# YuxiaWu/RAG4DyG

Hardware: AMD Instinct MI355X
Metric: query-seqs/sec encode+top-k over full pool (higher is better)
Workload: dtype f32 (f16x2 operands: two fp16 terms, three products, f32 accumulate)

## Files before the change

### rag4dyg_amd/build.py

```python
import os
import subprocess
import sys
from concurrent.futures import ThreadPoolExecutor

PKG = os.path.dirname(os.path.abspath(__file__))
CSRC = os.path.join(PKG, "csrc")
OBJ = os.path.join(PKG, "_build")
LIB = os.path.join(PKG, "librag4dyg_hip.so")
HIPCC = os.environ.get("HIPCC", "/opt/rocm/bin/hipcc")
FLAGS = ["-O3", "--offload-arch=gfx950", "-fPIC", "-std=c++17", "-Wall", "-Wno-unused-function"]


def sources():
    return sorted(os.path.join(CSRC, f) for f in os.listdir(CSRC) if f.endswith(".hip"))


def _deps_mtime():
    hdrs = [os.path.join(CSRC, f) for f in os.listdir(CSRC) if f.endswith(".h")]
    hdrs.append(os.path.join(os.path.dirname(PKG), "include", "r4d.h"))
    return max(os.path.getmtime(h) for h in hdrs)


def _compile(src, force, hdr_m):
    obj = os.path.join(OBJ, os.path.basename(src)[:-4] + ".o")
    if not force and os.path.exists(obj) and os.path.getmtime(obj) >= max(os.path.getmtime(src), hdr_m):
        return obj, False
    cmd = [HIPCC, *FLAGS, "-c", src, "-o", obj]
    r = subprocess.run(cmd, capture_output=True, text=True)
    if r.returncode != 0:
        raise RuntimeError(f"hipcc failed for {src}:\n{r.stdout}\n{r.stderr}")
    if r.stderr.strip():
        sys.stderr.write(r.stderr)
    return obj, True


HANDOFF_KERNELS = {"topk.hip": {"topk_chunk_kernelIfE": (4, 2), "topk_chunk_kernelIdE": (4, 2)},
                   "gemm_skinny.hip": {"gemm_skinny16_kernelILi2ELi0E": (2, 1), "gemm_skinny16_kernelILi3ELi0E": (2, 1)}}


def check_handoff_lowering(src):
    import re
    import tempfile
    names = HANDOFF_KERNELS[os.path.basename(src)]
    with tempfile.TemporaryDirectory() as td:
        asm = os.path.join(td, "k.s")
        r = subprocess.run([HIPCC, "-O3", "--offload-arch=gfx950", "-std=c++17", "--offload-device-only", "-S", src, "-o", asm],
                           capture_output=True, text=True)
        if r.returncode != 0:
            raise RuntimeError(f"hipcc -S failed for {src}:\n{r.stderr}")
        text = open(asm).read()
    for name, (want_st, want_ld) in names.items():
        m = re.search(r"^(_ZN3r4d\d+" + re.escape(name) + r"[^\n:]*):[^\n]*\n(.*?)s_endpgm", text, re.S | re.M)
        if not m:
            raise RuntimeError(f"hand-off check: kernel {name} not found in the assembly of {src}")
        body = m.group(2)
        stores = re.findall(r"global_store_dword(?:x2)? [^\n]*", body)
        loads_sc1 = [ln for ln in re.findall(r"global_load_dword(?:x2)? [^\n]*", body) if " sc1" in ln]
        stores_sc1 = [ln for ln in stores if " sc1" in ln]
        ticket = re.findall(r"global_atomic_add[^\n]*", body)
        if not ticket or len(stores_sc1) < want_st or len(loads_sc1) < want_ld:
            raise RuntimeError(f"hand-off check FAILED for {name}: {len(stores_sc1)} sc1 stores (want {want_st}), {len(loads_sc1)} sc1 loads (want {want_ld}), "
                               f"{len(ticket)} ticket atomics -- the relaxed agent-scope publish / consume of {os.path.basename(src)} "
                               "is no longer lowered to write-through / L1-bypassing instructions; use release / acquire there")


PACKED_F32_FILES = ("gemm_h2.hip", "attention_h2.hip")
PACKED_F32_FORMS = {
    "v_pk_mul_f32 V, V, S op_sel_hi:[1,0]", "v_pk_mul_f32 V, S, V op_sel_hi:[0,1]", "v_pk_mul_f32 V, V, S", "v_pk_mul_f32 V, S, V",
    "v_pk_fma_f32 V, V, S, V op_sel_hi:[1,0,1]", "v_pk_fma_f32 V, S, V, V op_sel_hi:[0,1,1]", "v_pk_fma_f32 V, V, S, V", "v_pk_fma_f32 V, S, V, V",
    "v_pk_fma_f32 V, V, S, V op_sel_hi:[1,0,1] neg_lo:[0,0,1] neg_hi:[0,0,1]",
    "v_pk_fma_f32 V, V, S, V op_sel_hi:[1,0,0] neg_lo:[1,0,0] neg_hi:[1,0,0]",
    "v_pk_fma_f32 V, S, V, V op_sel_hi:[0,1,1] neg_lo:[1,0,0] neg_hi:[1,0,0]",
    "v_pk_add_f32 V, V, S op_sel_hi:[1,0]", "v_pk_add_f32 V, S, V op_sel_hi:[0,1]",
}


def check_packed_f32_forms(src):
    import re
    import tempfile
    with tempfile.TemporaryDirectory() as td:
        asm = os.path.join(td, "k.s")
        r = subprocess.run([HIPCC, "-O3", "--offload-arch=gfx950", "-std=c++17", "--offload-device-only", "-S", src, "-o", asm],
                           capture_output=True, text=True)
        if r.returncode != 0:
            raise RuntimeError(f"hipcc -S failed for {src}:\n{r.stderr}")
        text = open(asm).read()
    seen = {}
    for ln in re.findall(r"^\s*(v_pk_(?:fma|mul|add)_f32 [^\n;]*)", text, re.M):
        if not re.search(r"\bs\[?\d", ln):
            continue
        form = re.sub(r"a\[[0-9:]+\]", "V", re.sub(r"v\[[0-9:]+\]", "V", re.sub(r"\bs\[[0-9:]+\]|\bs\d+\b", "S", ln))).strip()
        seen[form] = seen.get(form, 0) + 1
    new = {f: n for f, n in seen.items() if f not in PACKED_F32_FORMS}
    if new:
        raise RuntimeError(f"packed-fp32 census FAILED for {os.path.basename(src)}: operand forms with an SGPR source that "
                           f"tools/pk_fma_probe.hip has not verified on gfx950: {new} -- add the form to the probe, run it on the GPU, "
                           "then list it in rag4dyg_amd/build.py:PACKED_F32_FORMS (or pin that arithmetic scalar)")
    return seen


def build_library(force=False, verbose=True):
    os.makedirs(OBJ, exist_ok=True)
    hdr_m = _deps_mtime()
    with ThreadPoolExecutor(max_workers=4) as ex:
        res = list(ex.map(lambda s: _compile(s, force, hdr_m), sources()))
    objs = [o for o, _ in res]
    for src, (_o, compiled) in zip(sources(), res):
        if compiled and os.path.basename(src) in HANDOFF_KERNELS:
            check_handoff_lowering(src)
        if compiled and os.path.basename(src) in PACKED_F32_FILES:
            check_packed_f32_forms(src)
    stale = os.path.exists(LIB) and any(os.path.getmtime(o) > os.path.getmtime(LIB) for o in objs)
    if force or stale or any(c for _, c in res) or not os.path.exists(LIB):
        cmd = [HIPCC, "--offload-arch=gfx950", "-shared", "-fPIC", "-o", LIB, *objs]
        r = subprocess.run(cmd, capture_output=True, text=True)
        if r.returncode != 0:
            raise RuntimeError(f"link failed:\n{r.stdout}\n{r.stderr}")
        if verbose:
            print(f"built {LIB}")
    elif verbose:
        print(f"up to date: {LIB}")
    return LIB


if __name__ == "__main__":
    build_library(force="--force" in sys.argv)
```

### rag4dyg_amd/csrc/gemm_h2p_body.h

```cpp
    constexpr int NW = WGM * WGN;
    constexpr int WM = BM / WGM, WN = BN / WGN, TM = WM / 32, TN = WN / 32;
    constexpr int STAGE = (BM + BN) * 8;
    constexpr int NBUF = 3;
    constexpr int NGA = BM / 8 / NW, NGB = BN / 8 / NW;
    constexpr int NDMA = NGA + NGB;
    static_assert(BM == 128 && (BN == 256 || BN == 128) && TM >= 1 && TN >= 1 && (NGA == 2 || NGA == 4) && (NGB == 2 || NGB == 4 || NGB == 8), "tile");
    __shared__ u32x4 lds[NBUF * STAGE];

    static_assert(!ROWMAP || (EPI == EPI_H2WORDS && !OUT_LINES), "row-block map: the h2-word c_attn only");
    int m0, n0;
    if constexpr (ROWMAP) {
        const int tiles_m = rm.hdr[0] >> 2, tiles_n = (g.N + BN - 1) / BN, nreal = tiles_m * tiles_n;
        if ((int)blockIdx.x >= nreal) return;
        grouped_tile<BM, BN>(tiles_m, tiles_n, (int)blockIdx.x, nreal, m0, n0);
    } else {
        grouped_tile<BM, BN>(g.M, g.N, m0, n0);
    }
    const int nkt = g.K / 32;

    const int tid = threadIdx.x, lane = tid & 63, wid = tid >> 6;
    const int wm = wid / WGN, wn = wid % WGN;
    const int li = lane & 31, lh = lane >> 5;

    unsigned va[NGA], vb[NGB];
    const int lrow = lane >> 3, lslot = lane & 7;
#pragma unroll
    for (int i = 0; i < NGA; ++i) {
        const int r = (wid * NGA + i) * 8 + lrow;
        int arow;
        if constexpr (ROWMAP) {
            const int gr = rm.list[(m0 + r) >> 5] * 32 + (r & 31);
            arow = gr >= rm.m_tab ? rm.m_tab - 1 : (gr >= rm.m_real && gr < ((rm.m_real + 31) & ~31) ? rm.m_real - 1 : gr);
        } else {
            arow = min(m0 + r, g.M - 1);
        }
        va[i] = (unsigned)arow * (unsigned)(g.K * 4) + 16u * (unsigned)(lslot ^ ((r >> 1) & 7)) + 3072u - 1024u * (i & 3);
    }
#pragma unroll
    for (int i = 0; i < NGB; ++i) {
        const int r = (wid * NGB + i) * 8 + lrow;
        vb[i] = (unsigned)min(n0 + r, g.N - 1) * (unsigned)(g.K * 4) + 16u * (unsigned)(lslot ^ ((r >> 1) & 7)) + 3072u - 1024u * (i & 3);
    }
    const unsigned lds0 = __builtin_amdgcn_readfirstlane((unsigned)(size_t)lds);
    const unsigned wid_s = __builtin_amdgcn_readfirstlane((unsigned)wid);
    const unsigned dst_a = lds0 + (wid_s * NGA) * 1024u, dst_b = lds0 + ((unsigned)(BM / 8) + wid_s * NGB) * 1024u;
    const char* abase = reinterpret_cast<const char*>(Al) - 3072;
    const char* bbase = reinterpret_cast<const char*>(Bp) - 3072;
#define H2P_ISSUE(KT, STG)                                                                         \
    {                                                                                              \
        const unsigned so_ = (unsigned)(STG) * (unsigned)(STAGE * 16);                             \
        if constexpr (NGA == 4) h2p_dma4(abase + (size_t)(KT) * 128, va[0], va[1], va[2], va[3], dst_a + so_); \
        else h2p_dma2(abase + (size_t)(KT) * 128, va[0], va[1], dst_a + so_);                      \
        if constexpr (NGB == 8) {                                                                  \
            h2p_dma4(bbase + (size_t)(KT) * 128, vb[0], vb[1], vb[2], vb[3], dst_b + so_);          \
            h2p_dma4(bbase + (size_t)(KT) * 128, vb[4], vb[5], vb[6], vb[7], dst_b + so_ + 4096u);   \
        } else if constexpr (NGB == 4) h2p_dma4(bbase + (size_t)(KT) * 128, vb[0], vb[1], vb[2], vb[3], dst_b + so_); \
        else h2p_dma2(bbase + (size_t)(KT) * 128, vb[0], vb[1], dst_b + so_);                       \
    }

    const int fsw = (li >> 1) & 7;
    int f_off[2][2];
#pragma unroll
    for (int s_ = 0; s_ < 2; ++s_)
#pragma unroll
        for (int p = 0; p < 2; ++p) f_off[s_][p] = li * 8 + ((4 * p + 2 * s_ + lh) ^ fsw);
    const int fa_base = wm * WM * 8, fb_base = BM * 8 + wn * WN * 8;

    f32x16 acc0[TM][TN], acc1[TM][TN];
#pragma unroll
    for (int i = 0; i < TM; ++i)
#pragma unroll
        for (int j = 0; j < TN; ++j)
#pragma unroll
            for (int r = 0; r < 16; ++r) { acc0[i][j][r] = 0.f; acc1[i][j][r] = 0.f; }

#define H2P_MFMA(ACC, A_, B_, I_, J_) \
    ACC[I_][J_] = __builtin_amdgcn_mfma_f32_32x32x16_f16(__builtin_bit_cast(f16x8, A_), __builtin_bit_cast(f16x8, B_), ACC[I_][J_], 0, 0, 0);
    u32x4 fa[2][TM][2], fb[2][TN][2];
#define H2P_FRAGS(SET, STG, S)                                                                     \
    {                                                                                              \
        const u32x4* st_ = lds + (STG) * STAGE;                                                   \
                                        \
        _Pragma("unroll") for (int i = 0; i < TM; ++i) fa[SET][i][1] = st_[fa_base + i * 256 + f_off[S][1]]; \
        _Pragma("unroll") for (int j = 0; j < TN; ++j) fb[SET][j][0] = st_[fb_base + j * 256 + f_off[S][0]]; \
        _Pragma("unroll") for (int i = 0; i < TM; ++i) fa[SET][i][0] = st_[fa_base + i * 256 + f_off[S][0]]; \
        _Pragma("unroll") for (int j = 0; j < TN; ++j) fb[SET][j][1] = st_[fb_base + j * 256 + f_off[S][1]]; \
    }
#define H2P_MFMAS(SET)                                                                             \
    {                                                                                              \
        _Pragma("unroll") for (int i = 0; i < TM; ++i) _Pragma("unroll") for (int j = 0; j < TN; ++j) H2P_MFMA(acc1, fa[SET][i][1], fb[SET][j][0], i, j) \
        _Pragma("unroll") for (int i = 0; i < TM; ++i) _Pragma("unroll") for (int j = 0; j < TN; ++j) H2P_MFMA(acc0, fa[SET][i][0], fb[SET][j][0], i, j) \
        _Pragma("unroll") for (int i = 0; i < TM; ++i) _Pragma("unroll") for (int j = 0; j < TN; ++j) H2P_MFMA(acc1, fa[SET][i][0], fb[SET][j][1], i, j) \
    }

    H2P_ISSUE(0, 0)
    if (nkt > 1) { H2P_ISSUE(1, 1) h2p_wait_vm<NDMA>(); } else { h2p_wait_vm<0>(); }
    __syncthreads();
    H2P_FRAGS(0, 0, 0)

    constexpr int NMF = 3 * TM * TN, NFR = 2 * (TM + TN);
    static_assert(NMF >= NFR, "interleave");
#define H2P_ITER(CUR, NXT, WR)                                                                     \
    {                                                                                              \
        __builtin_amdgcn_sched_barrier(0);                                                         \
        const bool more_ = kt + 2 < nkt;                                                           \
        if (more_) H2P_ISSUE(kt + 2, WR)                                                           \
        H2P_FRAGS(1, CUR, 1)                                                                       \
        H2P_MFMAS(0)                                                                               \
        _Pragma("unroll") for (int m_ = 0; m_ < NMF; ++m_) {                                       \
            __builtin_amdgcn_sched_group_barrier(0x008, 1, 0);                                     \
            if (m_ < NFR) __builtin_amdgcn_sched_group_barrier(0x100, 1, 0);                       \
        }                                                                                          \
        __builtin_amdgcn_sched_barrier(0);                                                         \
        if (more_) h2p_wait_vm<NDMA>(); else h2p_wait_vm<0>();                                     \
        asm volatile("s_waitcnt lgkmcnt(0)\n\ts_barrier" ::: "memory");                            \
        H2P_FRAGS(0, NXT, 0)                                                                       \
        H2P_MFMAS(1)                                                                               \
        _Pragma("unroll") for (int m_ = 0; m_ < NMF; ++m_) {                                       \
            __builtin_amdgcn_sched_group_barrier(0x008, 1, 0);                                     \
            if (m_ < NFR) __builtin_amdgcn_sched_group_barrier(0x100, 1, 0);                       \
        }                                                                                          \
        __builtin_amdgcn_sched_barrier(0);                                                         \
    }
    int kt = 0;
    for (; kt + 2 < nkt; kt += 3) {
        H2P_ITER(0, 1, 2)
        { ++kt; H2P_ITER(1, 2, 0) }
        { ++kt; H2P_ITER(2, 0, 1) }
        kt -= 2;
    }
    if (kt < nkt) {
        H2P_ITER(0, 1, 2)
        if (kt + 1 < nkt) { ++kt; H2P_ITER(1, 2, 0) }
    }
#undef H2P_ITER
#undef H2P_FRAGS
#undef H2P_MFMAS
#undef H2P_MFMA
#undef H2P_ISSUE

    constexpr float UNS = H2_A_UNSCALE;
    float* __restrict__ C = Cg;
    const bool interior = ROWMAP || ((m0 + BM <= g.M) & (n0 + BN <= g.N));
    if constexpr (OUT_LINES) {
        static_assert(EPI == EPI_GELU, "line output: the c_fc epilogue only");
        unsigned char* __restrict__ L = reinterpret_cast<unsigned char*>(Cg);
        const long long row_bytes = (long long)g.N * 4;
        const bool odd = li & 1;
#pragma unroll
        for (int j = 0; j < TN; ++j) {
            const int colb = n0 + wn * WN + j * 32;
            const bool col_ok = colb + li < g.N;
            const float bias = (biasg && col_ok) ? biasg[colb + li] : 0.f;
#pragma unroll
            for (int i = 0; i < TM; ++i) {
#pragma unroll
                for (int r2 = 0; r2 < 16; r2 += 2) {
                    f32x2 v2 = {__builtin_fmaf(acc1[i][j][r2], H2_LO_UNSCALE, acc0[i][j][r2]) * UNS + bias,
                                __builtin_fmaf(acc1[i][j][r2 + 1], H2_LO_UNSCALE, acc0[i][j][r2 + 1]) * UNS + bias};
                    v2 = gelu_new2(v2);
                    const float vx = v2.x, vy = v2.y;
                    const float send = odd ? vx : vy;
                    const float recv = __builtin_bit_cast(float, __builtin_amdgcn_mov_dpp(__builtin_bit_cast(int, send), 0xB1, 0xF, 0xF, true));
                    const float c0 = odd ? recv : vx, c1 = odd ? vy : recv;
                    unsigned h, l;
                    split2_pair<true>(c0, c1, h, l);
                    const int r = r2 + (odd ? 1 : 0);
                    const int row = m0 + wm * WM + i * 32 + (r & 3) + 8 * (r >> 2) + 4 * lh;
                    if (interior || (row < g.M && col_ok)) {
                        unsigned* dst = reinterpret_cast<unsigned*>(L + (long long)row * row_bytes + (long long)(colb >> 5) * 128 + (li >> 1) * 4);
                        dst[0] = h;
                        dst[16] = l;
                    }
                }
            }
        }
        return;
    } else {
        if (interior) {
            const int lane_c = (((ROWMAP ? 0 : wm * WM) + 4 * lh) * g.ldc + wn * WN + li) * 4;
            const int lane_r = ((wm * WM + 4 * lh) * g.ldr + wn * WN + li) * 4;
            const __amdgpu_buffer_rsrc_t c_rsrc = __builtin_amdgcn_make_buffer_rsrc(
                C + (long long)(ROWMAP ? 0 : m0) * g.ldc + n0, 0, (((ROWMAP ? g.M : BM) - 1) * g.ldc + BN) * 4, 0x00020000);
            const __amdgpu_buffer_rsrc_t r_rsrc = __builtin_amdgcn_make_buffer_rsrc(
                const_cast<float*>(EPI == EPI_RESIDUAL ? residg + (long long)m0 * g.ldr + n0 : Cg), 0,
                EPI == EPI_RESIDUAL ? ((BM - 1) * g.ldr + BN) * 4 : 0, 0x00020000);
            const int kd = g.N / 3;
            const __amdgpu_buffer_rsrc_t kb_rsrc = __builtin_amdgcn_make_buffer_rsrc(
                (EPI == EPI_H2WORDS && g.kb_hd) ? g.kblk : reinterpret_cast<unsigned*>(Cg), 0,
                (EPI == EPI_H2WORDS && g.kb_hd) ? ((g.M + 31) / 32) * (kd * 128) : 0, 0x00020000);
            const int lane_kb = (li >> 3) * 1024 + ((li >> 2) & 1) * 512 + ((li & 3) + 4 * lh) * 16;
#pragma unroll
            for (int j = 0; j < TN; ++j) {
                const float bias = biasg ? biasg[n0 + wn * WN + j * 32 + li] : 0.f;
                const int colb = n0 + wn * WN + j * 32;
                const bool to_kb = EPI == EPI_H2WORDS && g.kb_hd && colb >= kd && colb < 2 * kd;
                const int kb_chunk = to_kb ? ((colb - kd) / g.kb_hd) * (g.kb_hd / 8) + ((colb - kd) % g.kb_hd) / 8 : 0;
#pragma unroll
                for (int i = 0; i < TM; ++i) {
                    const int blk = ROWMAP ? __builtin_amdgcn_readfirstlane(rm.list[(m0 + wm * WM + i * 32) >> 5]) : ((m0 + wm * WM + i * 32) >> 5);
                    const int kb_soff = (blk * (kd / 8) + kb_chunk) * 1024;
                    const int row_c = ROWMAP ? blk * 32 : i * 32;
                    float res[16];
                    if (EPI == EPI_RESIDUAL) {
#pragma unroll
                        for (int r = 0; r < 16; ++r)
                            res[r] = __builtin_bit_cast(float, __builtin_amdgcn_raw_buffer_load_b32(
                                r_rsrc, lane_r, ((i * 32 + (r & 3) + 8 * (r >> 2)) * g.ldr + j * 32) * 4, 0));
                    }
                    unsigned o[16];
#pragma unroll
                    for (int r2 = 0; r2 < 16; r2 += 2) {
                        f32x2 v2 = {__builtin_fmaf(acc1[i][j][r2], H2_LO_UNSCALE, acc0[i][j][r2]) * UNS + bias,
                                     __builtin_fmaf(acc1[i][j][r2 + 1], H2_LO_UNSCALE, acc0[i][j][r2 + 1]) * UNS + bias};
                        if (EPI == EPI_GELU) v2 = gelu_new2(v2);
                        else if (EPI == EPI_RESIDUAL) { v2.x += res[r2]; v2.y += res[r2 + 1]; }
                        const float vx = v2.x, vy = v2.y;
                        o[r2] = __builtin_bit_cast(unsigned int, vx); o[r2 + 1] = __builtin_bit_cast(unsigned int, vy);
                        if (EPI == EPI_H2WORDS) h2_words<true>(v2.x, v2.y, o[r2], o[r2 + 1]);
                    }
                    if (EPI == EPI_H2WORDS && to_kb) {
                        const bool o1 = li & 1, o2 = li & 2;
#pragma unroll
                        for (int a4 = 0; a4 < 16; a4 += 4) {
                            unsigned x0 = o[a4], x1 = o[a4 + 1], x2 = o[a4 + 2], x3 = o[a4 + 3];
                            {
                                const unsigned s01 = o1 ? x0 : x1, s23 = o1 ? x2 : x3;
                                const unsigned r01 = (unsigned)__builtin_amdgcn_mov_dpp((int)s01, 0xB1, 0xF, 0xF, true);
                                const unsigned r23 = (unsigned)__builtin_amdgcn_mov_dpp((int)s23, 0xB1, 0xF, 0xF, true);
                                if (o1) { x0 = r01; x2 = r23; } else { x1 = r01; x3 = r23; }
                            }
                            {
                                const unsigned s02 = o2 ? x0 : x2, s13 = o2 ? x1 : x3;
                                const unsigned r02 = (unsigned)__builtin_amdgcn_mov_dpp((int)s02, 0x4E, 0xF, 0xF, true);
                                const unsigned r13 = (unsigned)__builtin_amdgcn_mov_dpp((int)s13, 0x4E, 0xF, 0xF, true);
                                if (o2) { x0 = r02; x1 = r13; } else { x2 = r02; x3 = r13; }
                            }
                            const u32x4 slot = {x0, x1, x2, x3};
                            __builtin_amdgcn_raw_buffer_store_b128(slot, kb_rsrc, lane_kb, kb_soff + 2 * a4 * 16, 0);
                        }
                    } else {
#pragma unroll
                        for (int r = 0; r < 16; ++r)
                            __builtin_amdgcn_raw_buffer_store_b32(o[r], c_rsrc, lane_c, ((row_c + (r & 3) + 8 * (r >> 2)) * g.ldc + j * 32) * 4, 0);
                    }
                }
            }
            return;
        }
#pragma unroll
        for (int j = 0; j < TN; ++j) {
            const int col = n0 + wn * WN + j * 32 + li;
            const bool col_ok = col < g.N;
            const int colc = min(col, g.N - 1);
            const float bias = biasg ? biasg[colc] : 0.f;
#pragma unroll
            for (int i = 0; i < TM; ++i) {
#pragma unroll
                for (int r = 0; r < 16; ++r) {
                    const int row = m0 + wm * WM + i * 32 + (r & 3) + 8 * (r >> 2) + 4 * lh;
                    float v = __builtin_fmaf(acc1[i][j][r], H2_LO_UNSCALE, acc0[i][j][r]) * UNS + bias;
                    if (EPI == EPI_GELU) v = gelu_new1(v);
                    else if (EPI == EPI_RESIDUAL) v += residg[(long long)min(row, g.M - 1) * g.ldr + colc];
                    else if (EPI == EPI_H2WORDS) { unsigned w0, w1; h2_words<true>(v, 0.f, w0, w1); v = __builtin_bit_cast(float, w0); }
                    if (EPI == EPI_H2WORDS && g.kb_hd && col >= g.N / 3 && col < 2 * (g.N / 3)) {
                        const int kd = g.N / 3, e = (col - kd) % g.kb_hd, chunk = ((col - kd) / g.kb_hd) * (g.kb_hd / 8) + (e >> 3);
                        if (row < g.M)
                            g.kblk[((long long)(row >> 5) * (kd / 8) + chunk) * 256 + (((e >> 2) & 1) * 32 + (row & 31)) * 4 + (e & 3)] =
                                __builtin_bit_cast(unsigned, v);
                        continue;
                    }
                    if (row < g.M && col_ok) C[(long long)row * g.ldc + col] = v;
                }
            }
        }
    }
```

### rag4dyg_amd/csrc/h2.h

```cpp
#pragma once

namespace r4d {

typedef float h2_f32x2 __attribute__((ext_vector_type(2)));
typedef _Float16 h2_f16x2 __attribute__((ext_vector_type(2)));

constexpr float H2_A_PRESCALE = 0.25f;
constexpr float H2_A_UNSCALE = 4.0f;
constexpr float H2_LO_SCALE = 2048.0f;
constexpr float H2_LO_UNSCALE = 1.0f / 2048.0f;

template <bool PRESCALE>
__device__ __forceinline__ void split2_pair(float x0, float x1, unsigned& h, unsigned& l) {
    h2_f32x2 v = {x0, x1};
    if (PRESCALE) v = v * H2_A_PRESCALE;
    const h2_f16x2 hh = __builtin_convertvector(v, h2_f16x2);
    const h2_f32x2 hf = __builtin_convertvector(hh, h2_f32x2);
    const h2_f32x2 r = (v - hf) * H2_LO_SCALE;
    const h2_f16x2 ll = __builtin_convertvector(r, h2_f16x2);
    h = __builtin_bit_cast(unsigned, hh);
    l = __builtin_bit_cast(unsigned, ll);
}

template <bool PRESCALE>
__device__ __forceinline__ void h2_words(float x0, float x1, unsigned& w0, unsigned& w1) {
    unsigned h, l;
    split2_pair<PRESCALE>(x0, x1, h, l);
    w0 = __builtin_amdgcn_perm(l, h, 0x05040100u);
    w1 = __builtin_amdgcn_perm(l, h, 0x07060302u);
}
__device__ __forceinline__ void h2_forms(float x0, float x1, unsigned& f1_0, unsigned& f1_1, unsigned& f2_0, unsigned& f2_1) {
    unsigned h, l;
    split2_pair<false>(x0, x1, h, l);
    f1_0 = h & 0xffffu;
    f1_1 = h >> 16;
    f2_0 = __builtin_amdgcn_perm(h, l, 0x05040100u);
    f2_1 = __builtin_amdgcn_perm(h, l, 0x07060302u);
}

}
```

Baseline: 40350.

## Permute B rows so each lane owns adjacent column pairs; fuse hi/lo split via fma_mix

When TN==2, the B-tile rows are loaded in a permuted order so each lane's two 32-column subtiles hold adjacent output columns. This lets the epilogue emit 64-bit stores and vectorised residual loads, and run GELU on packed pairs. split2_pair now computes the fp16 low residual with inline-asm v_fma_mix instead of convert/subtract/convert; the old path stays for h2_words/h2_forms. A build-time assembly check guards the inline asm against missing wait-state hazards, and assembly generation is parallelised.

```diff
diff --git a/rag4dyg_amd/build.py b/rag4dyg_amd/build.py
--- a/rag4dyg_amd/build.py
+++ b/rag4dyg_amd/build.py
@@ -75,16 +75,10 @@
 }
 
 
-def check_packed_f32_forms(src):
+def check_packed_f32_forms(src, text=None):
     import re
-    import tempfile
-    with tempfile.TemporaryDirectory() as td:
-        asm = os.path.join(td, "k.s")
-        r = subprocess.run([HIPCC, "-O3", "--offload-arch=gfx950", "-std=c++17", "--offload-device-only", "-S", src, "-o", asm],
-                           capture_output=True, text=True)
-        if r.returncode != 0:
-            raise RuntimeError(f"hipcc -S failed for {src}:\n{r.stderr}")
-        text = open(asm).read()
+    if text is None:
+        text = _assembly(src)
     seen = {}
     for ln in re.findall(r"^\s*(v_pk_(?:fma|mul|add)_f32 [^\n;]*)", text, re.M):
         if not re.search(r"\bs\[?\d", ln):
@@ -99,6 +93,42 @@
     return seen
 
 
+H2_ASM_FILES = ("gemm_h2.hip", "gemm_h2p.hip", "attention_h2.hip", "encoder_ops.hip")
+TRANS_OPS = ("v_exp_", "v_log_", "v_rcp_", "v_rsq_", "v_sqrt_", "v_sin_", "v_cos_")
+
+
+def check_h2_asm_neighbours(text, name):
+    import re
+    ins = [ln.strip() for ln in text.split("\n") if re.match(r"\s+[a-z]", ln) and not ln.strip().startswith(".")]
+    regs = lambda tok: set(re.findall(r"\bv\d+\b", tok)) | {f"v{i}" for a, b in re.findall(r"v\[(\d+):(\d+)\]", tok) for i in range(int(a), int(b) + 1)}
+    bad = []
+    for i, ln in enumerate(ins):
+        if not ln.startswith("v_fma_mix"):
+            continue
+        ops = ln.split(None, 1)[1].split(",")
+        dst, srcs = regs(ops[0]), regs(",".join(ops[1:]))
+        if i and ins[i - 1].startswith(TRANS_OPS) and regs(ins[i - 1].split(None, 1)[1].split(",")[0]) & srcs:
+            bad.append((ins[i - 1], ln))
+        for nxt in ins[i + 1:i + 3]:
+            if "dpp" in nxt and regs(",".join(nxt.split(None, 1)[1].split(",")[1:])) & dst:
+                bad.append((ln, nxt))
+    if bad:
+        raise RuntimeError(f"h2.h asm check FAILED for {name}: an inline-asm v_fma_mix* stands where the compiler inserts no wait states: "
+                           f"{bad[:4]} -- let the asm read the result of a plain VALU instruction (csrc/h2.h)")
+    return sum(1 for ln in ins if ln.startswith("v_fma_mix"))
+
+
+def _assembly(src):
+    import tempfile
+    with tempfile.TemporaryDirectory() as td:
+        asm = os.path.join(td, "k.s")
+        r = subprocess.run([HIPCC, "-O3", "--offload-arch=gfx950", "-std=c++17", "--offload-device-only", "-S", src, "-o", asm],
+                           capture_output=True, text=True)
+        if r.returncode != 0:
+            raise RuntimeError(f"hipcc -S failed for {src}:\n{r.stderr}")
+        return open(asm).read()
+
+
 def build_library(force=False, verbose=True):
     os.makedirs(OBJ, exist_ok=True)
     hdr_m = _deps_mtime()
@@ -108,8 +138,13 @@
     for src, (_o, compiled) in zip(sources(), res):
         if compiled and os.path.basename(src) in HANDOFF_KERNELS:
             check_handoff_lowering(src)
-        if compiled and os.path.basename(src) in PACKED_F32_FILES:
-            check_packed_f32_forms(src)
+    todo = [src for src, (_o, compiled) in zip(sources(), res) if compiled and os.path.basename(src) in PACKED_F32_FILES + H2_ASM_FILES]
+    with ThreadPoolExecutor(max_workers=4) as ex:
+        for src, text in zip(todo, ex.map(_assembly, todo)):
+            if os.path.basename(src) in PACKED_F32_FILES:
+                check_packed_f32_forms(src, text)
+            if os.path.basename(src) in H2_ASM_FILES:
+                check_h2_asm_neighbours(text, os.path.basename(src))
     stale = os.path.exists(LIB) and any(os.path.getmtime(o) > os.path.getmtime(LIB) for o in objs)
     if force or stale or any(c for _, c in res) or not os.path.exists(LIB):
         cmd = [HIPCC, "--offload-arch=gfx950", "-shared", "-fPIC", "-o", LIB, *objs]
diff --git a/rag4dyg_amd/csrc/gemm_h2p_body.h b/rag4dyg_amd/csrc/gemm_h2p_body.h
--- a/rag4dyg_amd/csrc/gemm_h2p_body.h
+++ b/rag4dyg_amd/csrc/gemm_h2p_body.h
@@ -4,6 +4,7 @@
     constexpr int NBUF = 3;
     constexpr int NGA = BM / 8 / NW, NGB = BN / 8 / NW;
     constexpr int NDMA = NGA + NGB;
+    constexpr bool PAIRS = TN == 2 && !ROWMAP && EPI != EPI_H2WORDS;
     static_assert(BM == 128 && (BN == 256 || BN == 128) && TM >= 1 && TN >= 1 && (NGA == 2 || NGA == 4) && (NGB == 2 || NGB == 4 || NGB == 8), "tile");
     __shared__ u32x4 lds[NBUF * STAGE];
 
@@ -39,7 +40,8 @@
 #pragma unroll
     for (int i = 0; i < NGB; ++i) {
         const int r = (wid * NGB + i) * 8 + lrow;
-        vb[i] = (unsigned)min(n0 + r, g.N - 1) * (unsigned)(g.K * 4) + 16u * (unsigned)(lslot ^ ((r >> 1) & 7)) + 3072u - 1024u * (i & 3);
+        const int rs = PAIRS ? (r & ~63) + 2 * (r & 31) + ((r >> 5) & 1) : r;
+        vb[i] = (unsigned)min(n0 + rs, g.N - 1) * (unsigned)(g.K * 4) + 16u * (unsigned)(lslot ^ ((r >> 1) & 7)) + 3072u - 1024u * (i & 3);
     }
     const unsigned lds0 = __builtin_amdgcn_readfirstlane((unsigned)(size_t)lds);
     const unsigned wid_s = __builtin_amdgcn_readfirstlane((unsigned)wid);
@@ -146,6 +148,41 @@
         static_assert(EPI == EPI_GELU, "line output: the c_fc epilogue only");
         unsigned char* __restrict__ L = reinterpret_cast<unsigned char*>(Cg);
         const long long row_bytes = (long long)g.N * 4;
+        if constexpr (PAIRS) {
+            const int colp = n0 + wn * WN + 2 * li;
+            const bool col_ok = colp < g.N;
+            const float bias0 = (biasg && col_ok) ? biasg[colp] : 0.f, bias1 = (biasg && col_ok) ? biasg[colp + 1] : 0.f;
+            const int rows_in = min(BM, g.M - m0), cols_in = min(BN, g.N - n0);
+            const __amdgpu_buffer_rsrc_t l_rsrc = __builtin_amdgcn_make_buffer_rsrc(
+                L + (long long)m0 * row_bytes + (long long)n0 * 4, 0, ((rows_in - 1) * g.N + cols_in) * 4, 0x00020000);
+            const int lane_l = (wm * WM + 4 * lh) * (g.N * 4) + (wn * (WN / 32) + (li >> 4)) * 128 + (li & 15) * 4;
+#pragma unroll
+            for (int i = 0; i < TM; ++i) {
+#pragma unroll
+                for (int r2 = 0; r2 < 16; r2 += 2) {
+                    f32x2 va2 = {__builtin_fmaf(acc1[i][0][r2], H2_LO_UNSCALE, acc0[i][0][r2]) * UNS + bias0,
+                                 __builtin_fmaf(acc1[i][0][r2 + 1], H2_LO_UNSCALE, acc0[i][0][r2 + 1]) * UNS + bias0};
+                    f32x2 vb2 = {__builtin_fmaf(acc1[i][1][r2], H2_LO_UNSCALE, acc0[i][1][r2]) * UNS + bias1,
+                                 __builtin_fmaf(acc1[i][1][r2 + 1], H2_LO_UNSCALE, acc0[i][1][r2 + 1]) * UNS + bias1};
+                    va2 = gelu_new2(va2);
+                    vb2 = gelu_new2(vb2);
+                    const f32x2 sa = va2 * H2_A_PRESCALE, sb = vb2 * H2_A_PRESCALE;
+                    const f32x2 qa = va2 * (H2_A_PRESCALE * H2_LO_SCALE), qb = vb2 * (H2_A_PRESCALE * H2_LO_SCALE);
+                    unsigned h[2], l[2];
+                    split2_vq(sa.x, sb.x, qa.x, qb.x, h[0], l[0]);
+                    split2_vq(sa.y, sb.y, qa.y, qb.y, h[1], l[1]);
+#pragma unroll
+                    for (int t = 0; t < 2; ++t) {
+                        const int rr = i * 32 + ((r2 + t) & 3) + 8 * ((r2 + t) >> 2);
+                        if (interior || (m0 + wm * WM + rr + 4 * lh < g.M && col_ok)) {
+                            __builtin_amdgcn_raw_buffer_store_b32(h[t], l_rsrc, lane_l, rr * (g.N * 4), 0);
+                            __builtin_amdgcn_raw_buffer_store_b32(l[t], l_rsrc, lane_l + 64, rr * (g.N * 4), 0);
+                        }
+                    }
+                }
+            }
+            return;
+        }
         const bool odd = li & 1;
 #pragma unroll
         for (int j = 0; j < TN; ++j) {
@@ -177,7 +214,51 @@
         }
         return;
     } else {
-        if (interior) {
+        if constexpr (PAIRS) {
+            if (interior && ((g.ldc | (EPI == EPI_RESIDUAL ? g.ldr : 0)) & 1) == 0) {
+                const int cb = n0 + wn * WN;
+                const int lane_c = ((wm * WM + 4 * lh) * g.ldc + wn * WN + 2 * li) * 4;
+                const int lane_r = ((wm * WM + 4 * lh) * g.ldr + wn * WN + 2 * li) * 4;
+                const __amdgpu_buffer_rsrc_t c_rsrc = __builtin_amdgcn_make_buffer_rsrc(
+                    C + (long long)m0 * g.ldc + n0, 0, ((BM - 1) * g.ldc + BN) * 4, 0x00020000);
+                const __amdgpu_buffer_rsrc_t r_rsrc = __builtin_amdgcn_make_buffer_rsrc(
+                    const_cast<float*>(EPI == EPI_RESIDUAL ? residg + (long long)m0 * g.ldr + n0 : Cg), 0,
+                    EPI == EPI_RESIDUAL ? ((BM - 1) * g.ldr + BN) * 4 : 0, 0x00020000);
+                const float bias0 = biasg ? biasg[cb + 2 * li] : 0.f, bias1 = biasg ? biasg[cb + 2 * li + 1] : 0.f;
+#pragma unroll
+                for (int i = 0; i < TM; ++i) {
+                    u32x2 res[16];
+                    if (EPI == EPI_RESIDUAL) {
+#pragma unroll
+                        for (int r = 0; r < 16; ++r)
+                            res[r] = __builtin_amdgcn_raw_buffer_load_b64(r_rsrc, lane_r, ((i * 32 + (r & 3) + 8 * (r >> 2)) * g.ldr) * 4, 0);
+                    }
+                    unsigned o[2][16];
+#pragma unroll
+                    for (int r2 = 0; r2 < 16; r2 += 2) {
+#pragma unroll
+                        for (int j = 0; j < 2; ++j) {
+                            const float bias = j ? bias1 : bias0;
+                            f32x2 v2 = {__builtin_fmaf(acc1[i][j][r2], H2_LO_UNSCALE, acc0[i][j][r2]) * UNS + bias,
+                                         __builtin_fmaf(acc1[i][j][r2 + 1], H2_LO_UNSCALE, acc0[i][j][r2 + 1]) * UNS + bias};
+                            if (EPI == EPI_GELU) v2 = gelu_new2(v2);
+                            else if (EPI == EPI_RESIDUAL) {
+                                v2.x += __builtin_bit_cast(float, j ? res[r2].y : res[r2].x);
+                                v2.y += __builtin_bit_cast(float, j ? res[r2 + 1].y : res[r2 + 1].x);
+                            }
+                            const float vx = v2.x, vy = v2.y;
+                            o[j][r2] = __builtin_bit_cast(unsigned int, vx); o[j][r2 + 1] = __builtin_bit_cast(unsigned int, vy);
+                        }
+                    }
+#pragma unroll
+                    for (int r = 0; r < 16; ++r) {
+                        const u32x2 w = {o[0][r], o[1][r]};
+                        __builtin_amdgcn_raw_buffer_store_b64(w, c_rsrc, lane_c, ((i * 32 + (r & 3) + 8 * (r >> 2)) * g.ldc) * 4, 0);
+                    }
+                }
+                return;
+            }
+        } else if (interior) {
             const int lane_c = (((ROWMAP ? 0 : wm * WM) + 4 * lh) * g.ldc + wn * WN + li) * 4;
             const int lane_r = ((wm * WM + 4 * lh) * g.ldr + wn * WN + li) * 4;
             const __amdgpu_buffer_rsrc_t c_rsrc = __builtin_amdgcn_make_buffer_rsrc(
@@ -250,7 +331,7 @@
         }
 #pragma unroll
         for (int j = 0; j < TN; ++j) {
-            const int col = n0 + wn * WN + j * 32 + li;
+            const int col = n0 + wn * WN + (PAIRS ? 2 * li + j : j * 32 + li);
             const bool col_ok = col < g.N;
             const int colc = min(col, g.N - 1);
             const float bias = biasg ? biasg[colc] : 0.f;
diff --git a/rag4dyg_amd/csrc/h2.h b/rag4dyg_amd/csrc/h2.h
--- a/rag4dyg_amd/csrc/h2.h
+++ b/rag4dyg_amd/csrc/h2.h
@@ -10,8 +10,25 @@
 constexpr float H2_LO_SCALE = 2048.0f;
 constexpr float H2_LO_UNSCALE = 1.0f / 2048.0f;
 
+__device__ __forceinline__ void split2_vq(float v0, float v1, float q0, float q1, unsigned& h, unsigned& l) {
+    const h2_f32x2 v = {v0, v1};
+    h = __builtin_bit_cast(unsigned, __builtin_convertvector(v, h2_f16x2));
+    unsigned ll;
+    asm("v_fma_mixlo_f16 %0, %1, %2, %3 op_sel_hi:[1,0,0]" : "=v"(ll) : "v"(h), "s"(-H2_LO_SCALE), "v"(q0));
+    asm("v_fma_mixhi_f16 %0, %1, %2, %3 op_sel:[1,0,0] op_sel_hi:[1,0,0]" : "+v"(ll) : "v"(h), "s"(-H2_LO_SCALE), "v"(q1));
+    l = ll;
+}
+
 template <bool PRESCALE>
 __device__ __forceinline__ void split2_pair(float x0, float x1, unsigned& h, unsigned& l) {
+    const h2_f32x2 x = {x0, x1};
+    const h2_f32x2 v = PRESCALE ? x * H2_A_PRESCALE : x;
+    const h2_f32x2 q = x * ((PRESCALE ? H2_A_PRESCALE : 1.0f) * H2_LO_SCALE);
+    split2_vq(v.x, v.y, q.x, q.y, h, l);
+}
+
+template <bool PRESCALE>
+__device__ __forceinline__ void split2_pair_cvt(float x0, float x1, unsigned& h, unsigned& l) {
     h2_f32x2 v = {x0, x1};
     if (PRESCALE) v = v * H2_A_PRESCALE;
     const h2_f16x2 hh = __builtin_convertvector(v, h2_f16x2);
@@ -25,13 +42,13 @@
 template <bool PRESCALE>
 __device__ __forceinline__ void h2_words(float x0, float x1, unsigned& w0, unsigned& w1) {
     unsigned h, l;
-    split2_pair<PRESCALE>(x0, x1, h, l);
+    split2_pair_cvt<PRESCALE>(x0, x1, h, l);
     w0 = __builtin_amdgcn_perm(l, h, 0x05040100u);
     w1 = __builtin_amdgcn_perm(l, h, 0x07060302u);
 }
 __device__ __forceinline__ void h2_forms(float x0, float x1, unsigned& f1_0, unsigned& f1_1, unsigned& f2_0, unsigned& f2_1) {
     unsigned h, l;
-    split2_pair<false>(x0, x1, h, l);
+    split2_pair_cvt<false>(x0, x1, h, l);
     f1_0 = h & 0xffffu;
     f1_1 = h >> 16;
     f2_0 = __builtin_amdgcn_perm(h, l, 0x05040100u);
```

Measured after the change: 41020, median of 6. +1.7%, better.
